# jac99/Egonn

Hardware: AMD Instinct MI355X
Metric: LiDAR scans/sec (descriptor extraction), 50k-pt clouds @ 0.1m voxel (higher is better)
Workload: dtype f32

## Files before the change

egonn_amd/_lib.py:

```python
from __future__ import annotations

import ctypes as C
import os
from typing import List, Optional, Sequence

import torch

_HERE = os.path.dirname(os.path.abspath(__file__))
LIB_PATH = os.path.join(_HERE, "lib", "libegonn_hip.so")

QUANT_CARTESIAN, QUANT_POLAR = 0, 1
FLAG_DISABLE_GLOBAL, FLAG_DISABLE_LOCAL, FLAG_IGNORE_KP_REGRESSOR, FLAG_BF16 = 1, 2, 4, 8
FLAG_POOL_SPOC, FLAG_POOL_MAC = 16, 32
MINKFPN_SPLIT_TOPDOWN = 1
MINKFPN_BLOCKS = {'BasicBlock': 0, 'ECABasicBlock': 1}
MINKFPN_POOLING = {None: 0, 'GeM': 1, 'MAC': 2, 'SPoC': 3}

_P = C.c_void_p
_SIGS = [
    ("egonn_ctx_create", C.c_int, [C.POINTER(_P), C.c_int, C.c_int]),
    ("egonn_ctx_destroy", None, [_P]),
    ("egonn_last_error", C.c_char_p, []),
    ("egonn_debug_set_naive_conv", C.c_int, [_P, C.c_int]),
    ("egonn_debug_set_ksplit", C.c_int, [_P, C.c_int, C.c_int, C.c_int, C.c_int, C.c_int]),
    ("egonn_debug_keep_level_features", C.c_int, [_P, C.c_int]),
    ("egonn_debug_set_trace", C.c_int, [_P]),
    ("egonn_prepare_maps", C.c_int, [_P, C.c_int, _P]),
    ("egonn_debug_rowgroup_tables", C.c_int, [_P, C.c_int, C.c_int, _P, _P, C.c_int64, C.POINTER(C.c_int64), _P]),
    ("egonn_debug_rowgroup_perm", C.c_int, [_P, C.c_int, C.c_int, _P, C.c_int64, C.POINTER(C.c_int64), _P]),
    ("egonn_debug_radix_sort_scratch_bytes", C.c_int64, [C.c_int64, C.c_int]),
    ("egonn_debug_radix_sort", C.c_int, [_P, _P, _P, _P, C.c_int64, C.c_int, _P, _P, C.c_int, C.c_int, C.c_int,
                                         C.POINTER(C.c_int32), _P, C.c_int64, _P]),
    ("egonn_voxelize", C.c_int, [_P, _P, C.POINTER(C.c_int64), C.c_int, C.c_int, C.POINTER(C.c_float), _P]),
    ("egonn_ctx_reserve", C.c_int, [_P, C.c_int64, C.c_int, C.POINTER(C.c_int64)]),
    ("egonn_voxelize_device", C.c_int, [_P, _P, C.c_int64, _P, C.c_int, C.c_int, C.POINTER(C.c_float), _P]),
    ("egonn_plan_status", C.c_int, [_P, _P]),
    ("egonn_ctx_set_exact_fp32", C.c_int, [_P, C.c_int]),
    ("egonn_ctx_set_operand_autoscale", C.c_int, [_P, C.c_int]),
    ("egonn_level_capacity", C.c_int, [_P, C.c_int, C.POINTER(C.c_int64)]),
    ("egonn_graph_begin", C.c_int, [_P]),
    ("egonn_graph_end", C.c_int, [_P, C.POINTER(_P)]),
    ("egonn_graph_launch", C.c_int, [_P, _P]),
    ("egonn_graph_destroy", None, [_P]),
    ("egonn_coords_set", C.c_int, [_P, _P, C.c_int64, C.c_int, _P]),
    ("egonn_level_count", C.c_int, [_P, C.c_int, C.POINTER(C.c_int64)]),
    ("egonn_level_batch_offsets", C.c_int, [_P, C.c_int, C.POINTER(C.c_int64)]),
    ("egonn_level_coords", C.c_int, [_P, C.c_int, _P, _P]),
    ("egonn_input_index", C.c_int, [_P, _P, _P]),
    ("egonn_conv", C.c_int, [_P, C.c_int, C.c_int, C.c_int, _P, C.c_int, _P, C.c_int, _P, _P, C.c_int, _P, _P]),
    ("egonn_conv_transpose", C.c_int, [_P, C.c_int, _P, C.c_int, _P, C.c_int, _P, _P]),
    ("egonn_sparse_conv", C.c_int, [_P, C.c_int, C.c_int, _P, C.c_int, _P, C.c_int, C.c_int, _P, _P, C.c_int, _P, _P, _P]),
    ("egonn_map_groups", C.c_int, [_P, C.c_int, C.c_int, C.POINTER(C.c_int64), C.POINTER(C.c_int64), _P]),
    ("egonn_global_avg_pool", C.c_int, [_P, C.c_int, _P, C.c_int, _P, _P]),
    ("egonn_bn_fold", C.c_int, [_P, _P, _P, _P, C.c_float, C.c_int, _P, _P, _P]),
    ("egonn_block_tail", C.c_int, [_P, C.c_int, _P, _P, C.c_int, _P, C.c_int, _P, _P]),
    ("egonn_gem", C.c_int, [_P, C.c_int, _P, C.c_int, _P, _P, _P]),
    ("egonn_global_max_pool", C.c_int, [_P, C.c_int, _P, C.c_int, _P, _P]),
# ... 351 lines not shown

    def rowgroup_tables(self, map_kind: int, level_out: int, with_rows: bool = True):
        ng, _ = self.map_groups(map_kind, level_out)
        K = 27 if map_kind == 0 else 8
        gm = torch.empty(ng, dtype=torch.int32, device=self.device)
        sn = torch.empty((ng, K, 16), dtype=torch.int32, device=self.device) if with_rows else None
        n = C.c_int64()
        self._call(self.lib.egonn_debug_rowgroup_tables, self.h, map_kind, level_out, gm.data_ptr(),
                   sn.data_ptr() if with_rows else None, ng, C.byref(n))
        return gm, sn

    def rowgroup_perm(self, map_kind: int, level_out: int):
        ng, _ = self.map_groups(map_kind, level_out)
        pm = torch.empty((ng, 16), dtype=torch.int32, device=self.device)
        n = C.c_int64()
        self._call(self.lib.egonn_debug_rowgroup_perm, self.h, map_kind, level_out, pm.data_ptr(), ng, C.byref(n))
        return pm

    def set_naive_conv(self, on: bool):
        check(self.lib.egonn_debug_set_naive_conv(self.h, int(on)))

    def keep_level_features(self, on: bool):
        check(self.lib.egonn_debug_keep_level_features(self.h, int(bool(on))))

    def set_exact_fp32(self, on: bool):
        check(self.lib.egonn_ctx_set_exact_fp32(self.h, int(bool(on))))

    def set_operand_autoscale(self, on: bool):
        check(self.lib.egonn_ctx_set_operand_autoscale(self.h, int(bool(on))))

    def set_ksplit(self, map_class: int, level: int, kparts: int = -1, kw: int = -1, col_parts: int = -1):
        check(self.lib.egonn_debug_set_ksplit(self.h, int(map_class), int(level), int(kparts), int(kw), int(col_parts)))

    def global_avg_pool(self, level: int, x: torch.Tensor):
        x = _dev_f32(x, self.device)
        out = torch.empty((self.batch_size, x.shape[1]), dtype=torch.float32, device=self.device)
        self._call(self.lib.egonn_global_avg_pool, self.h, level, x.data_ptr(), x.shape[1], out.data_ptr())
        return out

    def bn_fold(self, bn: torch.nn.BatchNorm1d):
        c = bn.num_features
        w, b, rm, rv = (_dev_f32(t.detach(), self.device) for t in (bn.weight, bn.bias, bn.running_mean, bn.running_var))
        scale = torch.empty(c, dtype=torch.float32, device=self.device)
        shift = torch.empty(c, dtype=torch.float32, device=self.device)
        self._call(self.lib.egonn_bn_fold, w.data_ptr(), b.data_ptr(), rm.data_ptr(), rv.data_ptr(), float(bn.eps), c,
                   scale.data_ptr(), shift.data_ptr())
        return scale, shift

    def block_tail(self, level: int, x: torch.Tensor, residual: torch.Tensor, eca_weight: Optional[torch.Tensor] = None):
        x, residual = _dev_f32(x, self.device), _dev_f32(residual, self.device)
        assert x.shape == residual.shape == (self.level_count(level), x.shape[1])
        out = torch.empty_like(x)
        ew = None if eca_weight is None else _dev_f32(eca_weight.detach().reshape(-1), self.device)
        self._call(self.lib.egonn_block_tail, self.h, level, x.data_ptr(), residual.data_ptr(), x.shape[1], _ptr(ew),
                   0 if ew is None else ew.numel(), out.data_ptr())
        return out

    def se_gate(self, mean: torch.Tensor, w1, b1, w2, b2, want_hidden: bool = False):
        mean = _dev_f32(mean, self.device)
        w1, b1, w2, b2 = (_dev_f32(t.detach(), self.device) for t in (w1, b1, w2, b2))
        B, c = mean.shape
        h = w1.shape[0]
        assert w1.shape == (h, c) and w2.shape == (c, h) and b1.shape == (h,) and b2.shape == (c,)
        gate = torch.empty_like(mean)
        hid = torch.empty((B, h), dtype=torch.float32, device=self.device) if want_hidden else None
        self._call(self.lib.egonn_se_gate, mean.data_ptr(), w1.data_ptr(), b1.data_ptr(), w2.data_ptr(), b2.data_ptr(), B, c, h,
# ... 353 lines not shown
```

egonn_amd/csrc/common.h:

```cpp
#pragma once
#include <hip/hip_runtime.h>
#include <atomic>
#include <stdint.h>
#include <stdio.h>
#include <string.h>
#include <string>
#include <vector>

#define EGONN_MAX_LEVELS 10
#define EGONN_NUM_LEVELS 8
#define EGONN_MAX_BATCH 4096

#define API extern "C" __attribute__((visibility("default")))

namespace egonn {

void set_error(const char* fmt, ...);
#define EGONN_OK 0
#define EGONN_ERR_INVALID 1
#define EGONN_ERR_HIP 2
#define EGONN_ERR_RANGE 3
#define EGONN_ERR_STATE 4
#define EGONN_ERR_CAPACITY 5
#define EGONN_ERR_FP16_RANGE 6
// ... 165 lines not shown
  char filter[64] = "";
  std::vector<ProfRec> recs;
  std::vector<ProfRec> graph_recs;
  std::vector<hipEvent_t> pool;
  hipEvent_t get();
};

struct Switches {
  bool debug_sync;
  bool no_presplit;
  bool no_fused_down;
  bool no_fused_lateral;
  bool no_gated_k2s2;
  bool no_fused_ghead;
  bool no_split_heads;
  bool no_tail_split;
  bool no_task_order;
  bool flat_sort, sort_pairs;
  bool no_search67;
  int split_max_level;
  int split_max_level_k8;
  int split_cfg;
  int rg_first_pass;
  const char* ksplit[5];
};
const Switches& switches();

struct KsRule {
  int8_t kparts[2][EGONN_NUM_LEVELS];
  int8_t kw[2][EGONN_NUM_LEVELS];
  int8_t col_parts[EGONN_NUM_LEVELS];
};

struct Ctx {
  Profiler prof;
  KsRule ks_rule;
  uint16_t* conv0_lut = nullptr;
  unsigned long long* dev_pairs = nullptr;
  int device = 0;
  int coord_bits = 16;
  int split_max_level = 5;
  float* ks_part = nullptr;
  size_t ks_part_floats = 0;
  const void* sort_prezeroed = nullptr;
  int keep_level_features = 0;
  int operand_autoscale = 0;
  int conv_variant = 0;
  Arena plan_arena;
  Arena work_arena;
  Arena sort_arena;
  Plan plan;
  int32_t* host_counts = nullptr;
  int32_t* dev_counts = nullptr;
  int32_t* dev_flags = nullptr;
  int32_t* dev_fp16_flag = nullptr;
  bool reserved = false;
  int64_t reserve_points = 0;
  int reserve_batch = 0;
  int64_t reserve_cap[EGONN_MAX_LEVELS] = {};
  hipEvent_t ev0 = nullptr, ev1 = nullptr;
};

hipEvent_t* prof_kernel_events();
struct ProfScope {
  Ctx* ctx;
  hipStream_t st;
  int idx = -1;
  bool exact = false;
  bool in_graph = false;
  ProfScope(Ctx* c, hipStream_t s, const char* name, int kind, int level, int K, int cin, int cout, int es);
  ~ProfScope();
};

int ensure_level0_parent_table(Ctx* ctx, hipStream_t stream);
int ensure_rowgroups(Ctx* ctx, const int* kinds, const int* levels, int count, hipStream_t stream);
int rowgroup_cap_groups(const Plan& P, int level);

// ... 29 lines not shown
```

egonn_amd/csrc/kernels.h:

```cpp
#pragma once
#include "common.h"

namespace egonn {

const char* last_error();

bool sconv_rg_supported(int cin, int cout);
int pack_rg_weights(const float* W, int K, int cin, int cout, int bf16, int flip, int transpose, void* out,
                    hipStream_t stream);
extern unsigned long long* g_sconv_trace;
struct PackedKernel {
  const void* rg32 = nullptr;
  const void* rg16 = nullptr;
  const void* split = nullptr;
};
struct ConvCall {
  int kind = 0, level = 0;
  const void* in = nullptr; void* out = nullptr;
  int cin = 0, cout = 0, bf16 = 0;
  const float *scale = nullptr, *shift = nullptr;
  int relu = 0;
  float* psum = nullptr;
  const PackedKernel* packed = nullptr;
  const float* W = nullptr; float* scratch = nullptr; size_t scratch_floats = 0;
  int split_io = 0;
  const float *in2 = nullptr, *gate = nullptr;
  const float* residual = nullptr;
};
enum SconvRoute {
  ROUTE_PLAIN,
  ROUTE_SPLIT,
  ROUTE_TAIL_SPLIT,
  ROUTE_WG,
  ROUTE_DMA,
  ROUTE_RG
};
SconvRoute sconv_route(const Ctx* ctx, int kind, int level, int cin, int cout, int bf16);
bool sconv_split_arithmetic(const Ctx* ctx);
const char* sconv_kernel_name(const Ctx* ctx, int kind, int level, int cin, int cout, int bf16);
struct SconvLaunch {
  SconvRoute route = ROUTE_RG;
  const RowGroups* rg = nullptr;
  int64_t n_in_cap = 0;
  int64_t groups_hint = 0;
  const void* Wp = nullptr;
  int variant = 0;
  bool small = false;
  int32_t* flags = nullptr;
  int B = 0;
  int kparts = 1, kw = 0, col_parts = 0;
  float* part = nullptr; size_t part_floats = 0;
  uint32_t* in_absmax = nullptr; int64_t in_elems = 0;
};
int sconv_rg_forward(const ConvCall& c, const SconvLaunch& l, hipStream_t stream);
int dense_small_group3(const float* const* in, const int64_t* n, const int32_t* const* n_dev, const float* const* W, float* const* out,
                       hipStream_t stream);
int sconv_map(Ctx* ctx, const ConvCall& c, hipStream_t stream);
bool sconv_split_supported(int cin, int cout);
int pack_split_weights(const float* W, int K, int cin, int cout, int flip, int transpose, void* out, hipStream_t stream);
size_t split_weights_bytes(int K, int cin, int cout);
int sconv_split_forward(const ConvCall& c, const SconvLaunch& l, hipStream_t stream);
size_t sconv_split_part_floats(const RowGroups& rg, int cout, int kparts);
void sconv_ksplit_rule(const Ctx* ctx, int kind, int level, int* kparts, int* col_parts, int* kw);
void sconv_ksplit_defaults(KsRule* r);
size_t sconv_ksplit_scratch_floats(const Ctx* ctx);
static constexpr size_t SCONV_SCRATCH_FLOATS = (size_t)2 << 20;
int sconv_naive(const float* in, const int32_t* nbr, const float* W, const float* scale, const float* shift, int relu,
                float* out, int64_t n_out, int K, int cin, int cout, hipStream_t stream);
int conv0_lut_init(Ctx* ctx);
int conv0_k5_forward(Ctx* ctx, const float* feat, const float* W, int cout, const float* scale,
                     const float* shift, int relu, void* out, int out_bf16, hipStream_t stream, const void* wpk = nullptr);
int conv0_pack_unit(const float* W, void* wpk, hipStream_t stream);

enum Act { ACT_NONE = 0, ACT_RELU = 1, ACT_TANH = 2, ACT_SOFTPLUS = 3, ACT_SIGMOID = 4 };
int dense_forward(const float* in, int64_t n, int cin, const float* W, int w_out_in, int cout, const float* bias,
                  const float* scale, const float* shift, int act, const float* residual, float* out,
                  hipStream_t stream);
bool dense_gate_fusable(int64_t n, int cin, int cout);
int dense_forward_ex(const void* in, int in_bf16, int64_t n, int cin, const float* W, int w_out_in, int cout,
                     const float* bias, const float* scale, const float* shift, int act, const void* residual, int res_bf16,
                     void* out, int out_bf16, hipStream_t stream, const int32_t* n_dev = nullptr, const float* gate = nullptr,
                     const int32_t* boff = nullptr, int B = 0);
int bn_fold(const float* w, const float* b, const float* rm, const float* rv, float eps, int c, float* scale,
            float* shift, hipStream_t stream);
int gather_rows(const float* in, const int32_t* perm, int64_t n, int c, float* out, hipStream_t stream,
                const int32_t* n_dev = nullptr);
static constexpr int SEG_CHUNKS = 32;
int segment_partial_sums(const float* in, const int32_t* boff, int B, int c, int pow_mode, const float* p,
                         float* partial, hipStream_t stream);
int eca_apply(const float* x, const float* res, const float* partial, const int32_t* boff, int B, int64_t n, int c,
              const float* wconv, int ksize, float* out, hipStream_t stream);
int eca_gate_groups(const float* psum, const RowGroups& rg, const int32_t* boff, int B, int c, const float* wconv, int ksize,
                    float* gate, hipStream_t stream);
int eca_apply_gate(const void* x, const void* res, const float* gate, const int32_t* boff, int B, int64_t n, int c,
                   void* out, int bf16, hipStream_t stream);
int convert_bf16_to_f32(const void* in, int64_t n, float* out, hipStream_t stream);
int gem_finish(const float* partial, const int32_t* boff, int B, int c, const float* p, float* out,
               hipStream_t stream);
// ... 33 lines not shown
```

egonn_amd/csrc/model.hip:

```cpp
#include "model.h"

using namespace egonn;

namespace {

const int PLANES[7] = {32, 64, 64, 128, 128, 128, 128};
const int GLOBAL_CH = 128, GLOBAL_DIM = 256, LOCAL_CH = 64, LOCAL_DIM = 128;

}

API const char* egonn_last_error(void) { return last_error(); }

API int egonn_debug_set_naive_conv(egonn_ctx* c, int on) {
  EGONN_REQUIRE(c, EGONN_ERR_INVALID, "debug_set_naive_conv: null context");
  if (on >= 1000) { c->conv_variant = on; return EGONN_OK; }
  c->conv_variant = (on == 1) ? 3 : (on == 2 ? 1 : (on == 4 ? 2 : (on == 8 ? 4 : (on == 16 ? 5 : (on == 32 ? 6 : (on == 128 ? 9 : 0))))));
  return EGONN_OK;
}

API int egonn_debug_set_ksplit(egonn_ctx* c, int map_class, int level, int kparts, int kw, int col_parts) {
  EGONN_REQUIRE(c && (map_class == 0 || map_class == 1) && level >= 0 && level < EGONN_NUM_LEVELS, EGONN_ERR_INVALID,
                "debug_set_ksplit: bad argument");
  EGONN_REQUIRE(kparts <= 27 && kw <= 4 && col_parts <= 4, EGONN_ERR_INVALID, "debug_set_ksplit: kparts <= 27, kw <= 4, col_parts <= 4");
  if (kparts >= 0) c->ks_rule.kparts[map_class][level] = (int8_t)std::max(kparts, 1);
  if (kw >= 0) c->ks_rule.kw[map_class][level] = (int8_t)kw;
  if (col_parts >= 0) c->ks_rule.col_parts[level] = (int8_t)col_parts;
  return EGONN_OK;
}

API int egonn_ctx_create(egonn_ctx** out, int device, int coord_bits) {
  EGONN_REQUIRE(out != nullptr, EGONN_ERR_INVALID, "ctx_create: null out pointer");
  EGONN_REQUIRE(coord_bits >= 10 && coord_bits <= 16, EGONN_ERR_INVALID, "coord_bits=%d outside [10,16]", coord_bits);
  int ndev = 0;
  HIP_CHECK(hipGetDeviceCount(&ndev));
  EGONN_REQUIRE(device >= 0 && device < ndev, EGONN_ERR_INVALID, "device %d not present (%d HIP devices)", device, ndev);
  HIP_CHECK(hipSetDevice(device));
  hipDeviceProp_t prop;
  HIP_CHECK(hipGetDeviceProperties(&prop, device));
  EGONN_REQUIRE(strncmp(prop.gcnArchName, "gfx950", 6) == 0, EGONN_ERR_INVALID,
                "libegonn_hip is built for gfx950 (MI355X) only; device %d is %s", device, prop.gcnArchName);
  egonn_ctx* c = new egonn_ctx();
  c->device = device;
  c->coord_bits = coord_bits;
  const size_t hc = sizeof(int32_t) * (32 + (size_t)EGONN_NUM_LEVELS * (EGONN_MAX_BATCH + 1)) + sizeof(int64_t) * (EGONN_MAX_BATCH + 2);
  if (hipHostMalloc(reinterpret_cast<void**>(&c->host_counts), hc) != hipSuccess ||
      hipMalloc(reinterpret_cast<void**>(&c->dev_counts), sizeof(int32_t) * 32) != hipSuccess ||
      hipMalloc(reinterpret_cast<void**>(&c->dev_pairs), sizeof(unsigned long long) * 16) != hipSuccess) {
    set_error("ctx_create: allocation failed");
    delete c;
    return EGONN_ERR_HIP;
  }
  c->dev_flags = c->dev_counts + 16;
  c->dev_fp16_flag = c->dev_counts + 17;
  sconv_ksplit_defaults(&c->ks_rule);
  if (conv0_lut_init(c) != EGONN_OK) {
    egonn_ctx_destroy(c);
    return EGONN_ERR_HIP;
  }
  *out = c;
// ... 992 lines not shown
```

egonn_amd/csrc/sconv.hip:

```cpp
#include <stdlib.h>
#include <algorithm>
#include <type_traits>
#include <utility>

#include "common.h"
#include <hip/hip_ext.h>
#include "kernels.h"

namespace egonn {

typedef float f32x4 __attribute__((ext_vector_type(4)));
typedef short bf16x8_t __attribute__((ext_vector_type(8)));

__device__ static inline uint32_t f2bf(float a) {
  uint32_t u = __float_as_uint(a);
  u += 0x7FFFu + ((u >> 16) & 1u);
  return u >> 16;
}

__global__ void pack_rg_weights_kernel(const float* __restrict__ W, int K, int cin, int cout, int bf16, int flip,
                                       int transpose, void* __restrict__ out) {
  const int64_t e = (int64_t)blockIdx.x * blockDim.x + threadIdx.x;
  const int64_t per_k = (int64_t)cin * cout;
  if (e >= K * per_k) return;
// ... 1069 lines not shown
const char* sconv_kernel_name(const Ctx* ctx, int kind, int level, int cin, int cout, int bf16) {
  switch (sconv_route(ctx, kind, level, cin, cout, bf16)) {
    case ROUTE_SPLIT: return "sconv_split_kernel";
    case ROUTE_WG: return "sconv_wg_kernel";
    case ROUTE_DMA: return "sconv_dma_kernel";
    default: return "sconv_rg_kernel";
  }
}

void sconv_ksplit_defaults(KsRule* r) {
  static const KsRule rule = [] {
    KsRule q = {{{1, 1, 1, 1, 1, 1, 1, 1}, {1, 1, 1, 1, 1, 1, 1, 1}}, {{0, 0, 0, 2, 2, 2, 0, 0}, {0, 0, 0, 2, 2, 2, 0, 0}}, {0, 0, 0, 0, 0, 0, 0, 0}};
    auto parse = [](const char* e, int8_t* dst) {
      for (int l = 0; e && *e && l < EGONN_NUM_LEVELS; ++l) {
        dst[l] = (int8_t)atoi(e);
        e = strchr(e, ',');
        if (e) ++e;
      }
    };
    int8_t* const dst[5] = {q.kparts[0], q.kparts[1], q.kw[0], q.kw[1], q.col_parts};
    for (int i = 0; i < 5; ++i) parse(switches().ksplit[i], dst[i]);
    return q;
  }();
  *r = rule;
}
void sconv_ksplit_rule(const Ctx* ctx, int kind, int level, int* kparts, int* col_parts, int* kw) {
  const KsRule& rule = ctx->ks_rule;
  const int l = std::min(std::max(level, 0), EGONN_NUM_LEVELS - 1);
  const int K = kind == 0 ? 27 : 8, mc = kind == 0 ? 0 : 1;
  *kparts = std::min(std::max((int)rule.kparts[mc][l], 1), K);
  *col_parts = rule.col_parts[l];
  *kw = rule.kw[mc][l];
}
size_t sconv_ksplit_scratch_floats(const Ctx* ctx) {
  size_t need = 0;
  for (int kind = 0; kind <= 2; ++kind)
    for (int l = (kind == 2 ? 0 : 1); l < EGONN_NUM_LEVELS - (kind == 2 ? 1 : 0); ++l) {
      int kp, cp, kw;
      sconv_ksplit_rule(ctx, kind, l, &kp, &cp, &kw);
      if (kp > 1) need = std::max(need, (size_t)kp * rowgroup_cap_groups(ctx->plan, l) * 16 * 128);
    }
  return need;
}

static int route_kernel(const ConvCall& c, int K, bool split, hipStream_t stream, const void** Wp) {
  *Wp = !c.packed ? nullptr : (split ? c.packed->split : (c.bf16 ? c.packed->rg16 : c.packed->rg32));
  if (*Wp) return EGONN_OK;
  const size_t wn = split ? (split_weights_bytes(K, c.cin, c.cout) + 3) / 4 : (size_t)K * c.cin * c.cout;
  EGONN_REQUIRE(c.W && c.scratch && c.scratch_floats >= wn, EGONN_ERR_STATE, "sconv: no scratch to pack the kernel into");
  *Wp = c.scratch;
  return split ? pack_split_weights(c.W, K, c.cin, c.cout, 0, 0, c.scratch, stream)
               : pack_rg_weights(c.W, K, c.cin, c.cout, c.bf16, 0, 0, c.scratch, stream);
}

int sconv_map(Ctx* ctx, const ConvCall& c, hipStream_t stream) {
  Plan& P = ctx->plan;
  const int kind = c.kind, level = c.level;
  EGONN_REQUIRE(kind >= 0 && kind <= 2, EGONN_ERR_INVALID, "sconv: map kind %d", kind);
  const int lin = kind == 0 ? level : (kind == 1 ? level - 1 : level + 1);
  EGONN_REQUIRE(level >= 0 && level < EGONN_NUM_LEVELS && lin >= 0 && lin < EGONN_NUM_LEVELS, EGONN_ERR_INVALID,
                "sconv: level %d out of range for map kind %d", level, kind);
  Level& V = P.lv[level];
  if (V.n == 0) return EGONN_OK;
  const int K = kind == 0 ? 27 : 8;
  SconvLaunch l;
  l.route = sconv_route(ctx, kind, level, c.cin, c.cout, c.bf16);
  if (l.route == ROUTE_PLAIN) {
    EGONN_REQUIRE(!c.bf16, EGONN_ERR_INVALID, "sconv: bf16 feature maps need a 32/64/128/256-channel plan (%d->%d)", c.cin, c.cout);
    EGONN_REQUIRE(c.W, EGONN_ERR_INVALID, "sconv: the plain kernel needs the reference-layout kernel");
    if (kind == 2 && level == 0) EGONN_TRY(ensure_level0_parent_table(ctx, stream));
    const int32_t* nbr = kind == 0 ? V.nbr27 : (kind == 1 ? V.nbr8 : V.nbrT);
    EGONN_REQUIRE(!c.psum && !c.residual, EGONN_ERR_INVALID, "sconv: group sums / epilogue residuals are produced by the MFMA kernels only");
    return sconv_naive(reinterpret_cast<const float*>(c.in), nbr, c.W, c.scale, c.shift, c.relu, reinterpret_cast<float*>(c.out), V.n, K,
                       c.cin, c.cout, stream);
  }
  EGONN_TRY(ensure_rowgroups(ctx, &kind, &level, 1, stream));
  l.rg = kind == 0 ? &V.rg27 : (kind == 1 ? &V.rg8 : &V.rgT);
  l.n_in_cap = P.cap[lin]; l.groups_hint = l.rg->cap_groups;
  const bool split = l.route == ROUTE_SPLIT || l.route == ROUTE_TAIL_SPLIT;
  if (split) l.flags = ctx->dev_fp16_flag;
  if (l.route != ROUTE_SPLIT)
    EGONN_REQUIRE(c.split_io == 0 && !c.in2, EGONN_ERR_STATE,
                  "sconv: split-form maps and gated inputs are read and written by the split kernel only");
  EGONN_TRY(route_kernel(c, K, split, stream, &l.Wp));
  if (l.route != ROUTE_SPLIT) {
    l.variant = ctx->conv_variant;
    l.small = sconv_small_level(level, c.bf16);
    return sconv_rg_forward(c, l, stream);
  }
  sconv_ksplit_rule(ctx, kind, level, &l.kparts, &l.col_parts, &l.kw);
  if (c.in2) { l.kparts = 1; l.kw = 0; }
  if (c.cin < 64) l.kw = 0;
  l.variant = ctx->conv_variant >= 1000 ? ctx->conv_variant - 1000 : 0;
  l.B = P.batch; l.part = ctx->ks_part; l.part_floats = ctx->ks_part_floats;
  if (ctx->operand_autoscale) {
    l.in_absmax = reinterpret_cast<uint32_t*>(ctx->dev_counts + 24);
    l.in_elems = P.lv[lin].n * c.cin;
  }
  return sconv_split_forward(c, l, stream);
}

}
```

egonn_amd/csrc/sconv_split.hip:

```cpp
#include <stdlib.h>
#include <algorithm>
#include <type_traits>
#include <utility>

#include "common.h"
#include <hip/hip_ext.h>
#include "kernels.h"

namespace egonn {

typedef float f32x4 __attribute__((ext_vector_type(4)));
typedef float f32x2 __attribute__((ext_vector_type(2)));
typedef _Float16 f16x8_t __attribute__((ext_vector_type(8)));
typedef _Float16 f16x2_t __attribute__((ext_vector_type(2)));

__host__ __device__ static inline int sp_chan(int g, int e) { return e < 4 ? 4 * g + e : 16 + 4 * g + (e - 4); }

__global__ void split_absmax_kernel(const float* __restrict__ W, int64_t n, uint32_t* __restrict__ trailer) {
  const int64_t t = (int64_t)blockIdx.x * blockDim.x + threadIdx.x;
  float m = 0.f;
  for (int64_t i = t; i < n; i += (int64_t)gridDim.x * blockDim.x) {
    const float v = fabsf(W[i]);
    m = (v == v && v < INFINITY) ? fmaxf(m, v) : m;
  }
// ... 491 lines not shown
            acc[ns][1] += red[(((q - 1) * NW + wave) * NS * 2 + ns * 2 + 1) * 64 + lane];
          }
      }
    }
    if (live && kw == 0) {
      if constexpr (KS) {
        if (gm_all) {
          float* dst = p.part + (((int64_t)blockIdx.z * p.cap_groups + gw) * NSTOT + ns0) * 512 + lane * 4;
#pragma unroll
          for (int ns = 0; ns < NS; ++ns) {
            *reinterpret_cast<f32x4*>(dst + ns * 512) = acc[ns][0];
            *reinterpret_cast<f32x4*>(dst + ns * 512 + 256) = acc[ns][1];
          }
        }
      } else {
#pragma unroll
        for (int ns = 0; ns < NS; ++ns) split_epilogue<COUT>(p, acc[ns][0], acc[ns][1], ns0 + ns, orow, gw, l15, g4);
      }
    }
    if constexpr (TRACE) {
      asm volatile("s_waitcnt vmcnt(0)" ::: "memory");
      tr[10] = now();
      tr[11] = (unsigned long long)n_steps;
      if (lane == 0 && p.trace) {
        unsigned long long* o = p.trace + (int64_t)gw * 12;
#pragma unroll
        for (int q = 0; q < 12; ++q) o[q] = tr[q];
      }
    }
    __builtin_amdgcn_s_barrier();
  }
}

template <int COUT>
static int launch_split_reduce(const SplitArgs& a, int64_t groups_hint, hipStream_t stream, hipEvent_t ev_stop) {
  const dim3 grid((unsigned)groups_hint);
  if (ev_stop) hipExtLaunchKernelGGL((sconv_split_reduce_kernel<COUT>), grid, dim3(COUT * 2), 0, stream, nullptr, ev_stop, 0, a);
  else hipLaunchKernelGGL((sconv_split_reduce_kernel<COUT>), grid, dim3(COUT * 2), 0, stream, a);
  HIP_CHECK(hipGetLastError());
  return EGONN_OK;
}

template <int CIN, int COUT, int NW, int NSW, bool TRACE = false, bool GATED = false, bool KS = false, int KW = 1>
static int launch_split(const SplitArgs& a, int64_t groups_hint, hipStream_t stream) {
  using GEO = SplitGeom<NSW, NW, GATED, KW>;
  static AttrOnce attr_done;
  if (attr_done.need()) {
    HIP_CHECK(hipFuncSetAttribute(reinterpret_cast<const void*>(&sconv_split_kernel<CIN, COUT, NW, NSW, TRACE, GATED, KS, KW>),
                                  hipFuncAttributeMaxDynamicSharedMemorySize, 160 * 1024));
    attr_done.mark();
  }
  const int64_t ntask = cdiv(groups_hint, NW);
  int64_t gridx = std::min<int64_t>(std::max<int64_t>(ntask, 8), 1 << 20);
  gridx = (gridx + 7) / 8 * 8;
  const dim3 grid((unsigned)gridx, (unsigned)(COUT / 32 / NSW), (unsigned)a.kp_n);
  hipEvent_t* pev = prof_kernel_events();
  hipEvent_t ev_stop = nullptr;
  if (pev[0]) {
    ev_stop = pev[1];
    hipExtLaunchKernelGGL((sconv_split_kernel<CIN, COUT, NW, NSW, TRACE, GATED, KS, KW>), grid, dim3(NW * KW * 64), GEO::LDS_BYTES, stream,
                          pev[0], a.kp_n > 1 ? nullptr : pev[1], 0, a);
    pev[0] = pev[1] = nullptr;
  } else {
    hipLaunchKernelGGL((sconv_split_kernel<CIN, COUT, NW, NSW, TRACE, GATED, KS, KW>), grid, dim3(NW * KW * 64), GEO::LDS_BYTES, stream, a);
  }
  HIP_CHECK(hipGetLastError());
// ... 25 lines not shown
  a.w_bytes = (uint32_t)((uint64_t)rg.K * cin * cout * 4);
  a.K = rg.K; a.relu = c.relu ? 1 : 0; a.cap_groups = rg.cap_groups;
  a.flags = l.flags;
  a.res = c.residual;
  a.in_split = (c.split_io & 1) ? 1 : 0;
  if (l.in_absmax) {
    EGONN_REQUIRE(!(c.split_io & 1) && !c.in2 && l.in_elems > 0, EGONN_ERR_INVALID, "sconv(split): operand scale on a plain fp32 input only");
    HIP_CHECK(hipMemsetAsync(l.in_absmax, 0, 8, stream));
    hipLaunchKernelGGL(split_absmax_kernel, dim3((unsigned)std::min<int64_t>(cdiv(l.in_elems, 1024), 1024)), dim3(256), 0, stream, a.in, l.in_elems, l.in_absmax);
    a.in_maxbits = l.in_absmax + 1;
  }
  a.out_split = (c.split_io & 2) ? 1 : 0;
  if (l.kparts > 1) {
    EGONN_REQUIRE(l.kparts <= rg.K && !c.in2, EGONN_ERR_INVALID, "sconv(split): %d offset parts on a %d-slot map", l.kparts, rg.K);
    EGONN_REQUIRE(l.part && l.part_floats >= sconv_split_part_floats(rg, cout, l.kparts), EGONN_ERR_STATE,
                  "sconv(split): no scratch for the partial tiles of an offset-split launch");
    a.part = l.part;
    a.kp_n = l.kparts;
  }
  const int cfg = l.variant ? l.variant : (switches().split_cfg ? switches().split_cfg : 142);
  const bool trace = cfg >= 9000;
  int shape = trace ? cfg - 9000 : cfg;
  int parts_sel = 0;
  if (shape >= 500) { parts_sel = shape / 400; shape -= 400 * parts_sel; }
  const int ns_tot = cout / 32;
  int parts = 1;
  if (parts_sel > 0) parts = std::min(ns_tot, 1 << (parts_sel - 1));
  else if (l.col_parts > 0) parts = std::min(ns_tot, l.col_parts);
  else if (kw > 1) parts = std::max(1, ns_tot / 2);
  else if (ns_tot >= 2 && cdiv(groups_hint, 4) < 700) {
    parts = 2;
  }
  const int nsw = ns_tot / parts;
  if (c.in2) {
    EGONN_REQUIRE(cin == 32 && cout == 32 && c.gate && l.B >= 1 && !a.in_split && cfg == 142, EGONN_ERR_INVALID,
                  "sconv(split): the gated input exists for the 32->32 plan only");
    a.in2 = c.in2; a.gate = c.gate; a.B = l.B;
    return launch_split<32, 32, 4, 1, false, true>(a, groups_hint, stream);
  }
#define EGONN_SP_KW(CI, CO, NWW, NSWW, KWW)                                                               \
  if constexpr (SplitGeom<NSWW, NWW, false, KWW>::LDS_BYTES <= 160 * 1024) {                              \
    if (kw == KWW && a.kp_n > 1) return launch_split<CI, CO, NWW, NSWW, false, false, true, KWW>(a, groups_hint, stream);  \
    if (kw == KWW) return launch_split<CI, CO, NWW, NSWW, false, false, false, KWW>(a, groups_hint, stream); \
  }
#define EGONN_SP_LOCK1(CI, CO, NWW, NSWW)                                                                 \
  if (cin == CI && cout == CO && shape == 100 + NWW * 10 + 2 && nsw == NSWW && !trace) {                  \
    if constexpr (NWW == 4 && CI >= 64) {                                                                 \
      EGONN_SP_KW(CI, CO, NWW, NSWW, 2) EGONN_SP_KW(CI, CO, NWW, NSWW, 3) EGONN_SP_KW(CI, CO, NWW, NSWW, 4) \
      if (a.kp_n > 1) return launch_split<CI, CO, NWW, NSWW, false, false, true>(a, groups_hint, stream); \
    }                                                                                                     \
    EGONN_REQUIRE(a.kp_n == 1 && kw <= 1, EGONN_ERR_INVALID, "sconv(split): no offset-split instantiation for %d->%d (parts %d, kw %d)", cin, cout, a.kp_n, kw); \
    return launch_split<CI, CO, NWW, NSWW>(a, groups_hint, stream);                                       \
  }
#define EGONN_SP_LOCK(CI, CO, NWW)                                                                        \
  EGONN_SP_LOCK1(CI, CO, NWW, (CO / 32))                                                                  \
  if constexpr (CO >= 64) { EGONN_SP_LOCK1(CI, CO, NWW, (CO / 64)) }                                      \
  if constexpr (CO >= 128) { EGONN_SP_LOCK1(CI, CO, NWW, (CO / 128)) }
#define EGONN_SP_LOCK_TRACE(CI, CO, NWW)                                                                  \
  if (cin == CI && cout == CO && shape == 100 + NWW * 10 + 2 && trace) {                                  \
    a.trace = g_sconv_trace;                                                                              \
    return launch_split<CI, CO, NWW, (CO / 32), true>(a, groups_hint, stream);                            \
  }
  EGONN_SP_LOCK_TRACE(32, 32, 4) EGONN_SP_LOCK_TRACE(32, 32, 8) EGONN_SP_LOCK_TRACE(64, 64, 4)
  if (cin == 128 && cout == 128 && shape == 142 && trace) {
    a.trace = g_sconv_trace;
    return launch_split<128, 128, 4, 2, true>(a, groups_hint, stream);
  }
#define EGONN_SP_PLAN(CI, CO) EGONN_SP_LOCK(CI, CO, 8) EGONN_SP_LOCK(CI, CO, 4)
  EGONN_SP_PLAN(32, 32)
  EGONN_SP_PLAN(32, 64)
  EGONN_SP_PLAN(64, 64)
  EGONN_SP_PLAN(64, 128)
// ... 13 lines not shown
```

include/egonn_hip.h:

```cpp
#ifndef EGONN_HIP_H
#define EGONN_HIP_H

#include <stdint.h>

#ifdef __cplusplus
extern "C" {
#endif

typedef struct egonn_ctx egonn_ctx;
typedef struct egonn_model egonn_model;

enum { EGONN_QUANT_CARTESIAN = 0, EGONN_QUANT_POLAR = 1 };
enum { EGONN_STATUS_OK = 0, EGONN_STATUS_INVALID = 1, EGONN_STATUS_HIP = 2, EGONN_STATUS_RANGE = 3, EGONN_STATUS_STATE = 4,
       EGONN_STATUS_CAPACITY = 5,
       EGONN_STATUS_FP16_RANGE = 6 };
enum { EGONN_FLAG_DISABLE_GLOBAL = 1, EGONN_FLAG_DISABLE_LOCAL = 2, EGONN_FLAG_IGNORE_KP_REGRESSOR = 4,
       EGONN_FLAG_BF16 = 8,
       EGONN_FLAG_POOL_SPOC = 16, EGONN_FLAG_POOL_MAC = 32 };

int egonn_ctx_create(egonn_ctx** ctx, int device, int coord_bits);
void egonn_ctx_destroy(egonn_ctx* ctx);
const char* egonn_last_error(void);
int egonn_debug_set_naive_conv(egonn_ctx* ctx, int on);
int egonn_debug_set_ksplit(egonn_ctx* ctx, int map_class, int level, int kparts, int kw, int col_parts);
int egonn_debug_keep_level_features(egonn_ctx* ctx, int on);
int egonn_debug_set_trace(void* device_buffer);
int egonn_debug_rowgroup_tables(egonn_ctx* ctx, int map_kind, int level_out, uint32_t* gmask_out, int32_t* snbr_out,
                                int64_t capacity_groups, int64_t* n_groups, void* stream);
int egonn_debug_rowgroup_perm(egonn_ctx* ctx, int map_kind, int level_out, int32_t* perm_out, int64_t capacity_groups,
                              int64_t* n_groups, void* stream);
int64_t egonn_debug_radix_sort_scratch_bytes(int64_t n, int n_segments);
int egonn_debug_radix_sort(uint64_t* keys_in, uint32_t* vals_in, uint64_t* keys_out, uint32_t* vals_out, int64_t n, int nbits,
                           const int64_t* n_dev, const int64_t* seg_offsets, int n_segments, int idx_bits, int either_pair,
                           int32_t* result_pair, void* scratch, int64_t scratch_bytes, void* stream);

int egonn_voxelize(egonn_ctx* ctx, const float* points, const int64_t* scan_offsets, int batch_size, int quant_mode,
                   const float* step, void* stream);
int egonn_ctx_reserve(egonn_ctx* ctx, int64_t max_points, int batch_size, const int64_t* level_capacity);
int egonn_voxelize_device(egonn_ctx* ctx, const float* points, int64_t n_rows, const int64_t* scan_offsets_dev,
                          int batch_size, int quant_mode, const float* step, void* stream);
int egonn_plan_status(egonn_ctx* ctx, void* stream);
int egonn_ctx_set_exact_fp32(egonn_ctx* ctx, int on);
int egonn_ctx_set_operand_autoscale(egonn_ctx* ctx, int on);
int egonn_level_capacity(egonn_ctx* ctx, int level, int64_t* capacity);
typedef struct egonn_graph egonn_graph;
int egonn_graph_begin(void* stream);
int egonn_graph_end(void* stream, egonn_graph** graph);
int egonn_graph_launch(egonn_graph* graph, void* stream);
void egonn_graph_destroy(egonn_graph* graph);
int egonn_coords_set(egonn_ctx* ctx, const int32_t* coords, int64_t n, int batch_size, void* stream);

int egonn_level_count(egonn_ctx* ctx, int level, int64_t* n_rows);
int egonn_level_batch_offsets(egonn_ctx* ctx, int level, int64_t* offsets );
int egonn_level_coords(egonn_ctx* ctx, int level, int32_t* out, void* stream);
int egonn_input_index(egonn_ctx* ctx, int64_t* out , void* stream);

int egonn_conv(egonn_ctx* ctx, int level_in, int level_out, int kernel_size, const float* in, int cin,
// ... 259 lines not shown
```

Before: 22220.

## Add weight-resident persistent sparse-conv kernel for 32->32 level-1/2 convolutions

Adds a persistent kernel that loads the full 32->32 weight set into LDS once per workgroup, then has each wave loop over row-group tasks. Per-offset neighbor rows are double-buffered into LDS via buffer-load-to-LDS DMA while MFMA computes the previous offset. It targets the 8-slot convolutions at level 1 and the gated one at level 2, enabled by default through a mask of 6 (bit 1 is left off). The aim is to stop re-reading weights for every group and to hide gather latency, at the cost of heavy LDS use, lower occupancy and a fixed grid size.

Result: faster. 22560 (median of 6 runs) (+1.5%).

```diff
diff --git a/egonn_amd/_lib.py b/egonn_amd/_lib.py
--- a/egonn_amd/_lib.py
+++ b/egonn_amd/_lib.py
@@ -23,6 +23,7 @@
     ("egonn_last_error", C.c_char_p, []),
     ("egonn_debug_set_naive_conv", C.c_int, [_P, C.c_int]),
     ("egonn_debug_set_ksplit", C.c_int, [_P, C.c_int, C.c_int, C.c_int, C.c_int, C.c_int]),
+    ("egonn_debug_set_resident", C.c_int, [_P, C.c_int, C.c_int]),
     ("egonn_debug_keep_level_features", C.c_int, [_P, C.c_int]),
     ("egonn_debug_set_trace", C.c_int, [_P]),
     ("egonn_prepare_maps", C.c_int, [_P, C.c_int, _P]),
@@ -440,6 +441,9 @@
     def set_ksplit(self, map_class: int, level: int, kparts: int = -1, kw: int = -1, col_parts: int = -1):
         check(self.lib.egonn_debug_set_ksplit(self.h, int(map_class), int(level), int(kparts), int(kw), int(col_parts)))
 
+    def set_resident(self, mask: int = -1, max_workgroups: int = 0):
+        check(self.lib.egonn_debug_set_resident(self.h, int(mask), int(max_workgroups)))
+
     def global_avg_pool(self, level: int, x: torch.Tensor):
         x = _dev_f32(x, self.device)
         out = torch.empty((self.batch_size, x.shape[1]), dtype=torch.float32, device=self.device)
diff --git a/egonn_amd/csrc/common.h b/egonn_amd/csrc/common.h
--- a/egonn_amd/csrc/common.h
+++ b/egonn_amd/csrc/common.h
@@ -221,6 +221,8 @@
   int8_t col_parts[EGONN_NUM_LEVELS];
 };
 
+static constexpr int SCONV_RESIDENT_DEFAULT = 6;
+
 struct Ctx {
   Profiler prof;
   KsRule ks_rule;
@@ -232,6 +234,8 @@
   float* ks_part = nullptr;
   size_t ks_part_floats = 0;
   const void* sort_prezeroed = nullptr;
+  int resident_mask = SCONV_RESIDENT_DEFAULT;
+  int resident_wgs = 0;
   int keep_level_features = 0;
   int operand_autoscale = 0;
   int conv_variant = 0;
diff --git a/egonn_amd/csrc/kernels.h b/egonn_amd/csrc/kernels.h
--- a/egonn_amd/csrc/kernels.h
+++ b/egonn_amd/csrc/kernels.h
@@ -49,6 +49,7 @@
   int32_t* flags = nullptr;
   int B = 0;
   int kparts = 1, kw = 0, col_parts = 0;
+  int resident = 0, resident_wgs = 0;
   float* part = nullptr; size_t part_floats = 0;
   uint32_t* in_absmax = nullptr; int64_t in_elems = 0;
 };
@@ -64,6 +65,7 @@
 void sconv_ksplit_rule(const Ctx* ctx, int kind, int level, int* kparts, int* col_parts, int* kw);
 void sconv_ksplit_defaults(KsRule* r);
 size_t sconv_ksplit_scratch_floats(const Ctx* ctx);
+int sconv_resident_bit(int kind, int level, int cin, int cout, bool gated);
 static constexpr size_t SCONV_SCRATCH_FLOATS = (size_t)2 << 20;
 int sconv_naive(const float* in, const int32_t* nbr, const float* W, const float* scale, const float* shift, int relu,
                 float* out, int64_t n_out, int K, int cin, int cout, hipStream_t stream);
diff --git a/egonn_amd/csrc/model.hip b/egonn_amd/csrc/model.hip
--- a/egonn_amd/csrc/model.hip
+++ b/egonn_amd/csrc/model.hip
@@ -25,6 +25,14 @@
   if (kparts >= 0) c->ks_rule.kparts[map_class][level] = (int8_t)std::max(kparts, 1);
   if (kw >= 0) c->ks_rule.kw[map_class][level] = (int8_t)kw;
   if (col_parts >= 0) c->ks_rule.col_parts[level] = (int8_t)col_parts;
+  return EGONN_OK;
+}
+
+API int egonn_debug_set_resident(egonn_ctx* c, int mask, int max_workgroups) {
+  EGONN_REQUIRE(c && mask >= -1 && mask <= 7 && max_workgroups >= 0 && max_workgroups <= 65536, EGONN_ERR_INVALID,
+                "debug_set_resident: mask in [-1, 7], max_workgroups in [0, 65536]");
+  c->resident_mask = mask < 0 ? SCONV_RESIDENT_DEFAULT : mask;
+  c->resident_wgs = max_workgroups;
   return EGONN_OK;
 }
 
diff --git a/egonn_amd/csrc/sconv.hip b/egonn_amd/csrc/sconv.hip
--- a/egonn_amd/csrc/sconv.hip
+++ b/egonn_amd/csrc/sconv.hip
@@ -1125,6 +1125,13 @@
   *col_parts = rule.col_parts[l];
   *kw = rule.kw[mc][l];
 }
+int sconv_resident_bit(int kind, int level, int cin, int cout, bool gated) {
+  if (cin != 32 || cout != 32) return 0;
+  if (kind == 0 && level == 1 && !gated) return 1;
+  if (kind == 1 && level == 1 && !gated) return 2;
+  if (kind == 1 && level == 2 && gated) return 4;
+  return 0;
+}
 size_t sconv_ksplit_scratch_floats(const Ctx* ctx) {
   size_t need = 0;
   for (int kind = 0; kind <= 2; ++kind)
@@ -1185,6 +1192,9 @@
   if (c.in2) { l.kparts = 1; l.kw = 0; }
   if (c.cin < 64) l.kw = 0;
   l.variant = ctx->conv_variant >= 1000 ? ctx->conv_variant - 1000 : 0;
+  l.resident = (ctx->conv_variant == 0 && !ctx->operand_autoscale &&
+                (ctx->resident_mask & sconv_resident_bit(kind, level, c.cin, c.cout, c.in2 != nullptr)) != 0) ? 1 : 0;
+  l.resident_wgs = ctx->resident_wgs;
   l.B = P.batch; l.part = ctx->ks_part; l.part_floats = ctx->ks_part_floats;
   if (ctx->operand_autoscale) {
     l.in_absmax = reinterpret_cast<uint32_t*>(ctx->dev_counts + 24);
diff --git a/egonn_amd/csrc/sconv_split.hip b/egonn_amd/csrc/sconv_split.hip
--- a/egonn_amd/csrc/sconv_split.hip
+++ b/egonn_amd/csrc/sconv_split.hip
@@ -547,6 +547,263 @@
   }
 }
 
+template <int NW, bool GATED>
+struct ResidentGeom {
+  static constexpr int TBL = GATED ? 512 : 2048;
+  static constexpr int WAVE_LDS = TBL + 2 * 2048 + (GATED ? 2 * 2048 : 0);
+  static constexpr int lds_bytes(int K) { return K * 4096 + NW * WAVE_LDS; }
+};
+static_assert(ResidentGeom<8, false>::lds_bytes(27) <= 160 * 1024, "resident k=3 workgroup: LDS budget");
+static_assert(ResidentGeom<8, false>::lds_bytes(8) <= 80 * 1024, "resident 8-slot workgroups: two per CU");
+static_assert(ResidentGeom<12, true>::lds_bytes(8) <= 160 * 1024, "resident gated workgroup: LDS budget");
+
+template <int NW, bool GATED>
+__global__ __launch_bounds__(NW * 64) void sconv_split_resident_kernel(const SplitArgs p) {
+  using GEO = ResidentGeom<NW, GATED>;
+  constexpr int CIN = 32, COUT = 32, NOPS = GATED ? 4 : 2;
+  extern __shared__ __attribute__((aligned(1024))) char smem[];
+  typedef __attribute__((address_space(3))) char lds_char;
+  const int lane = threadIdx.x & 63;
+  const int wave = __builtin_amdgcn_readfirstlane(threadIdx.x >> 6);
+  const int l15 = lane & 15, g4 = lane >> 4;
+  const int K = p.K;
+  const float in_sc = p.in_maxbits ? split_scale_of(__builtin_amdgcn_readfirstlane((int)p.in_maxbits[0])) : 1.f;
+  char* const wl = smem + K * 4096 + wave * GEO::WAVE_LDS;
+  int32_t* const tbl = reinterpret_cast<int32_t*>(wl);
+  char* const ring = wl + GEO::TBL;
+  const uint32_t smem_addr = (uint32_t)(uintptr_t)(lds_char*)smem;
+  const uint32_t wl_addr = (uint32_t)(uintptr_t)(lds_char*)wl;
+  const uint32_t rd0 = wl_addr + GEO::TBL + (uint32_t)(l15 * 128 + ((g4 ^ (l15 & 7)) * 16));
+  const uint32_t rd1 = wl_addr + GEO::TBL + (uint32_t)(l15 * 128 + (((4 + g4) ^ (l15 & 7)) * 16));
+  const uint32_t tb0 = wl_addr + (uint32_t)((lane >> 3) * 4);
+  const uint32_t wrd = smem_addr + (uint32_t)(lane * 16);
+  const int dma_chunk = ((lane & 7) ^ (lane >> 3)) * 16;
+  const int w_lane = lane * 16;
+
+  const __amdgpu_buffer_rsrc_t a_rsrc =
+      __builtin_amdgcn_make_buffer_rsrc(const_cast<float*>(p.in), (short)(CIN * 4), (int)p.in_rows, 0x00020000);
+  const __amdgpu_buffer_rsrc_t w_rsrc = __builtin_amdgcn_make_buffer_rsrc(const_cast<void*>(p.Wsp), 0, (int)p.w_bytes, 0x00020000);
+  const __amdgpu_buffer_rsrc_t a2_rsrc =
+      __builtin_amdgcn_make_buffer_rsrc(const_cast<float*>(GATED ? p.in2 : p.in), (short)(CIN * 4), (int)p.in_rows, 0x00020000);
+
+  const int ngroups = __builtin_amdgcn_readfirstlane(min(p.meta[0], p.cap_groups));
+  const int ntask = (ngroups + 3) >> 2;
+  const int nx = (gridDim.x & 7) ? 1 : 8;
+  const int xcd = (int)blockIdx.x % nx, lb = (int)blockIdx.x / nx, nper = (int)gridDim.x / nx;
+  const int cpx = (ntask + nx - 1) / nx;
+  const int nslot = 4 * cpx, stride = nper * NW;
+  if (lb * NW >= nslot || xcd * cpx + ((lb * NW) >> 2) >= ntask) return;
+
+  for (int pc = wave; pc < K * 4; pc += NW)
+    __builtin_amdgcn_raw_ptr_buffer_load_lds(w_rsrc, (lds_char*)(smem + pc * 1024), 16, w_lane, pc * 1024, 0, 0);
+
+  struct Hdr {
+    int4 hv0, hv1;
+    int32_t orow;
+    uint32_t gm;
+    int gw;
+    f32x4 gq0, gq1;
+  };
+  auto task_at = [&](int s) {
+    const int tslot = xcd * cpx + (s >> 2);
+    if (s >= nslot || tslot >= ntask) return -1;
+    return p.order ? __builtin_amdgcn_readfirstlane(p.order[tslot]) : tslot;
+  };
+  int task_nx = task_at(lb * NW + wave);
+  auto fetch = [&](int& s, Hdr& h) {
+    h.gw = -1;
+    h.gm = 0;
+    for (; s < nslot; s += stride) {
+      const int task = task_nx;
+      task_nx = task_at(s + stride);
+      if (task < 0) { s = nslot; break; }
+      const int gw = task * 4 + (s & 3);
+      if (gw >= ngroups) continue;
+      h.gw = gw;
+      h.gm = p.gmask[gw];
+      const int n16 = K * 4;
+      const int4* src = reinterpret_cast<const int4*>(p.snbr + (int64_t)gw * K * 16);
+      h.hv0 = h.hv1 = make_int4(-1, -1, -1, -1);
+      if (lane < n16) h.hv0 = src[lane];
+      if (lane + 64 < n16) h.hv1 = src[lane + 64];
+      h.orow = p.perm[(int64_t)gw * 16 + l15];
+      if constexpr (GATED) {
+        int lo = 0, hi = p.B;
+        while (hi - lo > 1) {
+          const int mid = (lo + hi) >> 1;
+          if (p.meta[1 + mid] <= gw) lo = mid; else hi = mid;
+        }
+        h.gq0 = *reinterpret_cast<const f32x4*>(p.gate + (int64_t)lo * CIN + 4 * g4);
+        h.gq1 = *reinterpret_cast<const f32x4*>(p.gate + (int64_t)lo * CIN + 16 + 4 * g4);
+      }
+      s += stride;
+      return;
+    }
+  };
+
+  int s = lb * NW + wave;
+  Hdr cur, nxt;
+  fetch(s, cur);
+  asm volatile("s_waitcnt vmcnt(0)" ::: "memory");
+  __builtin_amdgcn_s_barrier();
+
+  auto mfma = [](const f32x4& wf, const f16x8_t& af, f32x4& c) {
+    c = __builtin_amdgcn_mfma_f32_16x16x32_f16(__builtin_bit_cast(f16x8_t, wf), af, c, 0, 0, 0);
+  };
+  uint32_t mk = 0;
+  int gw = -1, kA = 27, kB = 27, slot = 0;
+  int32_t orow = -1, i0 = -1, i1 = -1;
+  f32x4 gq0 = {0.f, 0.f, 0.f, 0.f}, gq1 = {0.f, 0.f, 0.f, 0.f};
+  f32x4 acc0 = {0.f, 0.f, 0.f, 0.f}, acc1 = {0.f, 0.f, 0.f, 0.f};
+  {
+    auto next_k = [&]() {
+      const int k = mk ? __builtin_ctz(mk) : 27;
+      mk &= mk - 1;
+      return k;
+    };
+    auto idx_read = [&](int k, int32_t& i0, int32_t& i1) {
+      if (k < 27) {
+        const uint32_t tb = tb0 + (uint32_t)(k * 64);
+        asm volatile("ds_read_b32 %0, %2\n\tds_read_b32 %1, %2 offset:32" : "=&v"(i0), "=&v"(i1) : "v"(tb) : "memory");
+      }
+    };
+    auto issue = [&](int slot, int k, int32_t i0, int32_t i1) {
+      if (k >= 27) return;
+      __builtin_amdgcn_struct_ptr_buffer_load_lds(a_rsrc, (lds_char*)(ring + slot * 2048), 16, i0, dma_chunk, 0, 0, 0);
+      __builtin_amdgcn_struct_ptr_buffer_load_lds(a_rsrc, (lds_char*)(ring + slot * 2048 + 1024), 16, i1, dma_chunk, 0, 0, 0);
+      if constexpr (GATED) {
+        __builtin_amdgcn_struct_ptr_buffer_load_lds(a2_rsrc, (lds_char*)(ring + 4096 + slot * 2048), 16, i0, dma_chunk, 0, 0, 0);
+        __builtin_amdgcn_struct_ptr_buffer_load_lds(a2_rsrc, (lds_char*)(ring + 4096 + slot * 2048 + 1024), 16, i1, dma_chunk, 0, 0, 0);
+      }
+    };
+    auto compute = [&](int slot, int k) {
+      f32x4 ra0, ra1, rb0, rb1, w[4];
+      const uint32_t r0 = rd0 + (uint32_t)(slot * 2048), r1 = rd1 + (uint32_t)(slot * 2048);
+      asm volatile("ds_read_b128 %0, %2\n\tds_read_b128 %1, %3" : "=&v"(ra0), "=&v"(ra1) : "v"(r0), "v"(r1) : "memory");
+      if constexpr (GATED) {
+        const uint32_t q0 = r0 + 4096u, q1 = r1 + 4096u;
+        asm volatile("ds_read_b128 %0, %2\n\tds_read_b128 %1, %3" : "=&v"(rb0), "=&v"(rb1) : "v"(q0), "v"(q1) : "memory");
+      }
+      const uint32_t wa = wrd + (uint32_t)(k * 4096);
+      asm volatile(
+          "ds_read_b128 %0, %4\n\t"
+          "ds_read_b128 %1, %4 offset:1024\n\t"
+          "ds_read_b128 %2, %4 offset:2048\n\t"
+          "ds_read_b128 %3, %4 offset:3072"
+          : "=&v"(w[0]), "=&v"(w[1]), "=&v"(w[2]), "=&v"(w[3])
+          : "v"(wa)
+          : "memory");
+      if constexpr (GATED) asm volatile("s_waitcnt lgkmcnt(0)" : "+v"(ra0), "+v"(ra1), "+v"(rb0), "+v"(rb1)::"memory");
+      else asm volatile("s_waitcnt lgkmcnt(0)" : "+v"(ra0), "+v"(ra1)::"memory");
+      asm volatile("s_waitcnt lgkmcnt(0)" : "+v"(w[0]), "+v"(w[1]), "+v"(w[2]), "+v"(w[3])::"memory");
+      f16x8_t ah, al;
+      if constexpr (GATED) {
+#pragma unroll
+        for (int u = 0; u < 4; ++u) {
+          ra0[u] = fmaxf(ra0[u] * gq0[u] + rb0[u], 0.f);
+          ra1[u] = fmaxf(ra1[u] * gq1[u] + rb1[u], 0.f);
+        }
+        split8h(ra0, ra1, ah, al);
+      } else if (p.in_split) { ah = __builtin_bit_cast(f16x8_t, ra0); al = __builtin_bit_cast(f16x8_t, ra1); }
+      else {
+        if (in_sc != 1.f) { ra0 *= in_sc; ra1 *= in_sc; }
+        split8h(ra0, ra1, ah, al);
+      }
+      __builtin_amdgcn_sched_barrier(0);
+      mfma(w[2], ah, acc0); mfma(w[3], ah, acc1);
+      mfma(w[0], al, acc0); mfma(w[1], al, acc1);
+      mfma(w[0], ah, acc0); mfma(w[1], ah, acc1);
+      __builtin_amdgcn_sched_barrier(0);
+    };
+
+    auto begin = [&]() {
+      while (cur.gw >= 0 && !((uint32_t)__builtin_amdgcn_readfirstlane((int)cur.gm) >> 31)) {
+        fetch(s, nxt);
+        cur = nxt;
+      }
+      if (cur.gw < 0) return false;
+      gw = cur.gw;
+      orow = cur.orow;
+      mk = (uint32_t)__builtin_amdgcn_readfirstlane((int)cur.gm) & 0x07FFFFFFu;
+      if constexpr (GATED) { gq0 = cur.gq0; gq1 = cur.gq1; }
+      {
+        int4* dst = reinterpret_cast<int4*>(tbl);
+        if (lane < K * 4) dst[lane] = cur.hv0;
+        if (lane + 64 < K * 4) dst[lane + 64] = cur.hv1;
+      }
+      __builtin_amdgcn_fence(__ATOMIC_RELEASE, "wavefront");
+      __builtin_amdgcn_wave_barrier();
+      __builtin_amdgcn_fence(__ATOMIC_ACQUIRE, "wavefront");
+      asm volatile("s_waitcnt lgkmcnt(0)" ::: "memory");
+      fetch(s, nxt);
+      kA = next_k();
+      kB = next_k();
+      slot = 0;
+      idx_read(kA, i0, i1);
+      asm volatile("s_waitcnt lgkmcnt(0)" : "+v"(i0), "+v"(i1)::"memory");
+      issue(0, kA, i0, i1);
+      idx_read(kB, i0, i1);
+      asm volatile("s_waitcnt lgkmcnt(0)" : "+v"(i0), "+v"(i1)::"memory");
+      issue(1, kB, i0, i1);
+      return true;
+    };
+
+    bool have = begin();
+    while (have) {
+      const int e_gw = gw;
+      const int32_t e_orow = orow;
+      acc0 = acc1 = (f32x4){0.f, 0.f, 0.f, 0.f};
+      while (kA < 27) {
+        const int kC = next_k();
+        idx_read(kC, i0, i1);
+        if (kB < 27) {
+          if constexpr (GATED) asm volatile("s_waitcnt vmcnt(4)" ::: "memory");
+          else asm volatile("s_waitcnt vmcnt(2)" ::: "memory");
+        } else {
+          asm volatile("s_waitcnt vmcnt(0)" ::: "memory");
+        }
+        static_assert(NOPS == (GATED ? 4 : 2), "the counted waits above");
+        __builtin_amdgcn_sched_barrier(0);
+        compute(slot, kA);
+        asm volatile("s_waitcnt lgkmcnt(0)" : "+v"(i0), "+v"(i1)::"memory");
+        issue(slot, kC, i0, i1);
+        __builtin_amdgcn_sched_barrier(0);
+        kA = kB; kB = kC; slot ^= 1;
+      }
+      const f32x4 e0 = acc0, e1 = acc1;
+      cur = nxt;
+      have = begin();
+      split_epilogue<COUT>(p, e0, e1, 0, e_orow, e_gw, l15, g4);
+    }
+  }
+}
+
+template <int NW, bool GATED>
+static int launch_split_resident(const SplitArgs& a, int64_t groups_hint, int max_workgroups, hipStream_t stream) {
+  using GEO = ResidentGeom<NW, GATED>;
+  const int lds = GEO::lds_bytes(a.K);
+  EGONN_REQUIRE(lds <= 160 * 1024 && a.K * 64 <= GEO::TBL, EGONN_ERR_INVALID, "sconv(split, resident): K = %d, %d bytes of LDS", a.K, lds);
+  static AttrOnce attr_done;
+  if (attr_done.need()) {
+    HIP_CHECK(hipFuncSetAttribute(reinterpret_cast<const void*>(&sconv_split_resident_kernel<NW, GATED>),
+                                  hipFuncAttributeMaxDynamicSharedMemorySize, 160 * 1024));
+    attr_done.mark();
+  }
+  int64_t gridx = (a.K > 8 || GATED) ? 256 : 512;
+  gridx = std::min<int64_t>(gridx, (std::max<int64_t>(cdiv(groups_hint, NW), 8) + 7) / 8 * 8);
+  if (max_workgroups > 0) gridx = std::min<int64_t>(max_workgroups, 1 << 16);
+  const dim3 grid((unsigned)gridx);
+  hipEvent_t* pev = prof_kernel_events();
+  if (pev[0]) {
+    hipExtLaunchKernelGGL((sconv_split_resident_kernel<NW, GATED>), grid, dim3(NW * 64), lds, stream, pev[0], pev[1], 0, a);
+    pev[0] = pev[1] = nullptr;
+  } else {
+    hipLaunchKernelGGL((sconv_split_resident_kernel<NW, GATED>), grid, dim3(NW * 64), lds, stream, a);
+  }
+  HIP_CHECK(hipGetLastError());
+  return EGONN_OK;
+}
+
 template <int COUT>
 static int launch_split_reduce(const SplitArgs& a, int64_t groups_hint, hipStream_t stream, hipEvent_t ev_stop) {
   const dim3 grid((unsigned)groups_hint);
@@ -638,12 +895,21 @@
     parts = 2;
   }
   const int nsw = ns_tot / parts;
+  const bool resident = !trace && (shape == 183 || (l.resident && cfg == 142));
+  if (resident)
+    EGONN_REQUIRE(cin == 32 && cout == 32 && a.kp_n == 1 && kw <= 1 && (rg.K == 27 || rg.K == 8), EGONN_ERR_INVALID,
+                  "sconv(split): the weight-resident form exists for the unsplit 32->32 plan only (%d->%d, K %d)", cin, cout, rg.K);
   if (c.in2) {
-    EGONN_REQUIRE(cin == 32 && cout == 32 && c.gate && l.B >= 1 && !a.in_split && cfg == 142, EGONN_ERR_INVALID,
+    EGONN_REQUIRE(cin == 32 && cout == 32 && c.gate && l.B >= 1 && !a.in_split && (cfg == 142 || resident), EGONN_ERR_INVALID,
                   "sconv(split): the gated input exists for the 32->32 plan only");
     a.in2 = c.in2; a.gate = c.gate; a.B = l.B;
+    if (resident) {
+      EGONN_REQUIRE(rg.K == 8, EGONN_ERR_INVALID, "sconv(split): the gated resident form exists for the 8-slot maps");
+      return launch_split_resident<12, true>(a, groups_hint, l.resident_wgs, stream);
+    }
     return launch_split<32, 32, 4, 1, false, true>(a, groups_hint, stream);
   }
+  if (resident) return launch_split_resident<8, false>(a, groups_hint, l.resident_wgs, stream);
 #define EGONN_SP_KW(CI, CO, NWW, NSWW, KWW)                                                               \
   if constexpr (SplitGeom<NSWW, NWW, false, KWW>::LDS_BYTES <= 160 * 1024) {                              \
     if (kw == KWW && a.kp_n > 1) return launch_split<CI, CO, NWW, NSWW, false, false, true, KWW>(a, groups_hint, stream);  \
diff --git a/include/egonn_hip.h b/include/egonn_hip.h
--- a/include/egonn_hip.h
+++ b/include/egonn_hip.h
@@ -23,6 +23,7 @@
 const char* egonn_last_error(void);
 int egonn_debug_set_naive_conv(egonn_ctx* ctx, int on);
 int egonn_debug_set_ksplit(egonn_ctx* ctx, int map_class, int level, int kparts, int kw, int col_parts);
+int egonn_debug_set_resident(egonn_ctx* ctx, int mask, int max_workgroups);
 int egonn_debug_keep_level_features(egonn_ctx* ctx, int on);
 int egonn_debug_set_trace(void* device_buffer);
 int egonn_debug_rowgroup_tables(egonn_ctx* ctx, int map_kind, int level_out, uint32_t* gmask_out, int32_t* snbr_out,
```
